# UDC-GAC/pRIblast

Measured on NVIDIA B200. Metric: db-step accessibility throughput, higher is better.
Workload: dtype f32

## Files before the change

### priblast_b200/csrc/acc_kernels.cu

```cuda
#include <cuda_runtime.h>
#include <nvtx3/nvToolsExt.h>

#include <algorithm>
#include <cstdio>
#include <cstdlib>
#include <cstring>
#include <new>
#include <numeric>
#include <string>
#include <vector>

#include "../../include/priblast_acc.h"
#include "acc_core.h"
#include "acc_exact.h"
#include "acc_tables.h"
#include "acc_tile.h"
#include "acc_wide.h"

using namespace prib;

namespace {

struct NvtxRange {
  explicit NvtxRange(const char *name) { nvtxRangePushA(name); }
  ~NvtxRange() { nvtxRangePop(); }
};

constexpr int kThreads = 128;
constexpr int kScanWarps = 4;
constexpr int kFp32MaxSpan = kMaxSpan;
#ifndef PRIB_TC32
#define PRIB_TC32 640
#endif
#ifndef PRIB_TC64
#define PRIB_TC64 288
#endif
template <typename real> struct TileChain { static constexpr bool value = sizeof(real) == 4 && PRIB_CHAIN != 0; };
template <typename real> struct TileMaxThreads { static constexpr int value = sizeof(real) == 4 ? PRIB_TC32 : PRIB_TC64; };

constexpr int kProgBytes = 128 + 16;
template <typename real>
__host__ __device__ constexpr size_t tile_smem_bytes() {
  return ((size_t)kTilePad + (size_t)kTileRows * TileMaxThreads<real>::value) * sizeof(real) +
         (Core<real>::kHotBytes + TileMaxThreads<real>::value + kMaxSpan + 16 + 15) / 16 * 16
         + kProgBytes;
}

__device__ __forceinline__ unsigned smem_u32(const void *p) { return (unsigned)__cvta_generic_to_shared(p); }
__device__ __forceinline__ void tma_bar_init(unsigned long long *bar, unsigned count) {
  asm volatile("mbarrier.init.shared::cta.b64 [%0], %1;" ::"r"(smem_u32(bar)), "r"(count) : "memory");
  asm volatile("fence.mbarrier_init.release.cluster;" ::: "memory");
}
__device__ __forceinline__ void tma_bar_expect(unsigned long long *bar, unsigned bytes) {
  asm volatile("mbarrier.arrive.expect_tx.shared::cta.b64 _, [%0], %1;" ::"r"(smem_u32(bar)), "r"(bytes) : "memory");
}
__device__ __forceinline__ void tma_bar_wait(unsigned long long *bar, unsigned parity) {
  asm volatile(
      "{\n"
      ".reg .pred p;\n"
      "TMA_WAIT:\n"
      "mbarrier.try_wait.parity.shared::cta.b64 p, [%0], %1;\n"
// ... 28 lines not shown
    asm volatile("st.volatile.shared.b32 [%0], %1;" ::"r"((unsigned)__cvta_generic_to_shared(prog + warp)), "r"(value) : "memory");
}
__device__ __forceinline__ void prog_wait_smem(const int *prog, int warp, int need) {
  const unsigned addr = (unsigned)__cvta_generic_to_shared(prog + warp);
  int v;
  do {
    asm volatile("ld.volatile.shared.b32 %0, [%1];" : "=r"(v) : "r"(addr) : "memory");
  } while (v < need);
}
#else
__device__ __forceinline__ void prog_signal_smem(int *prog, int warp, int lane, int value) { prog_signal(prog, warp, lane, value); }
__device__ __forceinline__ void prog_wait_smem(const int *prog, int warp, int need) { prog_wait(prog, warp, need); }
#endif
struct StepSignal {
  int *prog;
  int warp, lane, value;
  bool release;
  __device__ __forceinline__ void operator()() const {
    if (release) prog_signal(prog, warp, lane, value);
    else prog_signal_smem(prog, warp, lane, value);
  }
};

template <typename real, int PAR >
__global__ void __launch_bounds__(TileMaxThreads<real>::value, 1)
k_inside_tile(typename Core<real>::Ctx c, int TX, long long ntiles, real *scratch) {
  constexpr bool CH = TileChain<real>::value;
  typedef Tile<real> TL;
  constexpr int TC = TileMaxThreads<real>::value;
  extern __shared__ __align__(16) unsigned char smem_raw[];
  const int t = threadIdx.x, W = c.W, warp = t >> 5, lane = t & 31;
  constexpr int NW = TC / 32;
  real *base = reinterpret_cast<real *>(smem_raw) + kTilePad;
  unsigned char *stab = smem_raw + ((size_t)kTilePad + (size_t)kTileRows * TC) * sizeof(real);
  uint8_t *sS = stab + Core<real>::kHotBytes;
  const typename Core<real>::SmallTables &T = *reinterpret_cast<const typename Core<real>::SmallTables *>(stab);
  real *scrM1 = scratch + (size_t)blockIdx.x * 2 * (W + 4) * TC;
  real *scrM2 = scrM1 + (size_t)(W + 4) * TC;
  const typename TL::InSmem sm = TL::carve_in(base, TC, sS);
  const int dfirst = TL::first_group(W);
  int *prog = reinterpret_cast<int *>(smem_raw + tile_smem_bytes<real>() - kProgBytes);
  if (t < 32) prog[t] = 0;
  {
    unsigned long long *tbar = reinterpret_cast<unsigned long long *>(prog + 32);
    if (t == 0) {
      tma_bar_init(tbar, 1);
      tma_bar_expect(tbar, (unsigned)Core<real>::kHotBytes);
      tma_copy_g2s(stab, c.T, (unsigned)Core<real>::kHotBytes, tbar);
    }
    __syncthreads();
    tma_bar_wait(tbar, 0);
  }
  int ebase = 0;
  __syncthreads();
  for (long long tile = blockIdx.x; tile < ntiles; tile += gridDim.x) {
    typename TL::Geo ge;
    ge.g0 = tile * TX;
    ge.TC = TC;
    ge.TX = TX;
    ge.H = W + 1;
    __syncthreads();
    for (int k = t; k < kTileRows * TC; k += TC) base[k] = 0;
    for (int k = t; k < TC + 8; k += TC) sS[k] = (ge.g0 + k < c.NC) ? c.S[ge.g0 + k] : 0;
    typename TL::ColState cs;
    TL::col_state(c, ge.g0 + t, cs);
    __syncthreads();
    int ev = ebase, grp = 0;
    typename TL::Chain ch;
    if constexpr (CH) TL::clear(ch);
    for (int d0 = dfirst; d0 <= W + 1; d0 += kTT, ++grp) {
      real gs[kTT], mb[kTT], bs[kTT];
      real *xch = sm.xch + (grp & 1) * kTT * TC;
      if (warp + 1 < NW) prog_wait(prog, warp + 1, ev);
      if constexpr (CH) {
        if (warp >= 2) prog_wait(prog, warp - 2, ev - kEvPerGroup);
        TL::template inside_deep_chain<PAR, TC>(T, ge, sm, scrM1, scrM2, t, d0, ch, xch, mb, bs);
      } else {
        TL::template inside_deep<TC>(T, ge, sm, scrM1, scrM2, t, d0, gs, mb, bs);
      }
      prog_signal_smem(prog, warp, lane, ++ev);
#pragma unroll
      for (int k = 0; k < kTT; ++k) {
        ++ev;
        if (d0 + k >= kTurn) {
          if ((k > 0 || CH) && warp + 1 < NW) prog_wait_smem(prog, warp + 1, ev - 1);
          if (CH && warp + 2 < NW) prog_wait_smem(prog, warp + 2, ev - 1 - k);
          if (warp > 0) prog_wait_smem(prog, warp - 1, ev - kEvSlackIn);
          TL::template inside_shallow<TC>(c, T, ge, sm, scrM1, scrM2, t, cs, d0 + k, CH ? xch[k * TC + t] : gs[k], mb[k],
                                          bs[k], StepSignal{prog, warp, lane, ev, k == kTT - 1});
        } else {
          prog_signal(prog, warp, lane, ev);
        }
      }
    }
    ebase = ev;
  }
}

template <typename real>
__global__ void __launch_bounds__(TileMaxThreads<real>::value, 1)
k_outside_tile(typename Core<real>::Ctx c, int TX, long long ntiles, real *scratch) {
  constexpr bool CH = TileChain<real>::value;
  typedef Tile<real> TL;
  constexpr int TC = TileMaxThreads<real>::value;
  extern __shared__ __align__(16) unsigned char smem_raw[];
  const int t = threadIdx.x, W = c.W, warp = t >> 5, lane = t & 31;
  constexpr int NW = TC / 32;
  real *pad = reinterpret_cast<real *>(smem_raw);
  real *base = pad + kTilePad;
  unsigned char *stab = smem_raw + ((size_t)kTilePad + (size_t)kTileRows * TC) * sizeof(real);
  const typename Core<real>::SmallTables &T = *reinterpret_cast<const typename Core<real>::SmallTables *>(stab);
  uint8_t *sS = stab + Core<real>::kHotBytes;
  real *scrBif = scratch + (size_t)blockIdx.x * 2 * (W + 4) * TC;
  const typename TL::OutSmem sm = TL::carve_out(base, TC, sS);
  const int dlast = TL::first_group(W);
  int *prog = reinterpret_cast<int *>(smem_raw + tile_smem_bytes<real>() - kProgBytes);
  if (t < 32) prog[t] = 0;
  {
    unsigned long long *tbar = reinterpret_cast<unsigned long long *>(prog + 32);
    if (t == 0) {
      tma_bar_init(tbar, 1);
      tma_bar_expect(tbar, (unsigned)Core<real>::kHotBytes);
      tma_copy_g2s(stab, c.T, (unsigned)Core<real>::kHotBytes, tbar);
    }
    __syncthreads();
    tma_bar_wait(tbar, 0);
  }
  int ebase = 0;
  __syncthreads();
  for (long long tile = blockIdx.x; tile < ntiles; tile += gridDim.x) {
    typename TL::Geo ge;
    ge.g0 = tile * TX;
    ge.TC = TC;
    ge.TX = TX;
    ge.H = W + 1;
    __syncthreads();
    for (int k = t; k < kTilePad + kTileRows * TC; k += TC) pad[k] = 0;
    for (int k = t; k < TC + W + kOutBaseTail; k += TC) {
      const long long col = ge.g0 - ge.H - kOutBaseLead + k;
      sS[k] = (col >= 0 && col < c.NC) ? c.S[col] : 0;
    }
    typename TL::ColState cs;
    TL::col_state(c, ge.g0 - ge.H + t, cs);
    __syncthreads();
    int slot = (W + 1) % kRingOut;
    int ev = ebase, grp = 0;
    typename TL::Chain ch;
    if constexpr (CH) TL::clear(ch);
    for (int d0 = W + 1; d0 >= dlast + kTT - 1; d0 -= kTT, ++grp) {
      typename TL::OutDeep o;
      real *xch = sm.xch + (grp & 1) * kTT * TC;
      if (warp > 0) prog_wait(prog, warp - 1, ev);
      if constexpr (CH) {
        if (warp + 2 < NW) prog_wait(prog, warp + 2, ev - kEvPerGroup);
        TL::template outside_deep_chain<TC>(c, T, ge, sm, scrBif, t, cs, d0, slot, ch, xch, o);
      } else {
        TL::template outside_deep<TC>(c, T, ge, sm, scrBif, t, cs, d0, slot, o);
      }
      prog_signal_smem(prog, warp, lane, ++ev);
#pragma unroll
      for (int k = 0; k < kTT; ++k) {
        ++ev;
        if (d0 - k >= kTurn) {
          if ((k > 0 || CH) && warp > 0) prog_wait_smem(prog, warp - 1, ev - 1);
          if (CH && warp >= 2) prog_wait_smem(prog, warp - 2, ev - 1 - k);
          if (warp + 1 < NW) prog_wait_smem(prog, warp + 1, ev - kEvSlackOut);
          TL::template outside_shallow<TC>(c, T, ge, sm, scrBif, t, cs, d0 - k, slot, CH ? xch[k * TC + t] : o.gs[k],
                                           o.bs[k], o.bm1[k], o.ks[k], StepSignal{prog, warp, lane, ev, k == kTT - 1});
        } else {
          prog_signal(prog, warp, lane, ev);
        }
        slot = slot == 0 ? kRingOut - 1 : slot - 1;
      }
    }
    ebase = ev;
  }
}

template <int BYTES>
__device__ __forceinline__ void cp_async_or_zero(void *smem_dst, const void *gsrc, bool pred) {
  const unsigned dst = (unsigned)__cvta_generic_to_shared(smem_dst);
  const int src_bytes = pred ? BYTES : 0;
  asm volatile("cp.async.ca.shared.global [%0], [%1], %2, %3;" ::"r"(dst), "l"(gsrc), "n"(BYTES), "r"(src_bytes) : "memory");
}

template <typename real, bool ALPHA>
__device__ void warp_scan(const typename Core<real>::Ctx &c, int sq, double *ring, real *wbuf, const double *usm,
                          int lane) {
  const int L = c.seq_len[sq], W = c.W;
  const long long off = c.seq_off[sq];
  const double kBig = Core<real>::kScanBig, kLn2 = 0.6931471805599453094;
// ... 291 lines not shown
}

struct prib_ctx {
  prib_acc_params prm{};
  int W = 70, delta = 5;
  bool use_fp32 = true;
  cudaStream_t own_stream = nullptr, stream = nullptr;
  cudaEvent_t ev0 = nullptr, ev1 = nullptr, evk0 = nullptr, evk1 = nullptr;
  cudaEvent_t evp[PRIB_NUM_PHASES + 1] = {};
  bool phases_pending = false, kernel_timed = true, stage_timed = true;
  struct Pipelined {
    bool on = false, launched = false;
    const char *const *seq = nullptr;
    long long fpos = 0;
  } pipe;
  Engine<float> e32;
  Engine<double> e64;
  ExactEngine *ex = nullptr;
  long long ex_max_cols = 0;
  WideEngine *wide = nullptr;
  float *d_log = nullptr;
  int grid_tiles = 0;
  char *d_tile_scratch = nullptr;
  char *d_state = nullptr;
  long long state_cap_bytes = 0;
  long long state_budget = 0;
  long long budget_default = 0, budget_long = 0;
  void set_budget(long long budget) {
    e64.max_cols = budget / state_bytes_per_column(W, 8) / 32 * 32;
    e32.max_cols = budget / state_bytes_per_column(W, 4) / 32 * 32;
    ex_max_cols = budget / exact_state_bytes_per_column(W) / 32 * 32;
    state_budget = budget;
  }
  std::vector<Batch> batches;
  std::vector<int32_t> seq_len;
  std::vector<long long> seq_pos;
  unsigned char *h_arena = nullptr;
  size_t h_arena_cap = 0, h_arena_used = 0;
  unsigned char *h_meta = nullptr;
  size_t h_meta_cap = 0, h_meta_used = 0;
  size_t n_batches = 0;
  float *d_out = nullptr;
  long long out_floats = 0, out_cap = 0;
  bool staged = false, computed = false;
  float *h_stage = nullptr;
  long long h_stage_floats = 0;
// ... 233 lines not shown
    }
    raw_begin += bytes;
    ++used;
  }
  *n_live = used;
  return PRIB_OK;
}

template <typename real>
int run_batch(prib_ctx *c, const Batch &b, bool timed) {
  Engine<real> &e = engine<real>(c);
  if (timed && settle_phases(c) != PRIB_OK) return PRIB_ECUDA;
  const long long used = state_bytes_per_column(c->W, sizeof(real)) * b.NC;
  if (ensure_state(c, used) != PRIB_OK) return PRIB_ECUDA;
  const typename Core<real>::Ctx k = make_ctx<real>(c, b);
  cudaStream_t st = c->stream;
  if (used > c->cnt.dp_state_bytes_used) c->cnt.dp_state_bytes_used = used;
  if (timed) CU(cudaEventRecord(c->evp[0], st));
  CU(cudaMemsetAsync(b.d_flags, 0, sizeof(int32_t) * (size_t)std::max(b.n, 1), st));
  const unsigned grid = (unsigned)((b.NC + kThreads - 1) / kThreads);
  if (timed) CU(cudaEventRecord(c->evp[1], st));
  NvtxRange nvtx_batch("prib:device_batch");
  nvtxRangePushA("prib:inside");
  const int TX = e.TC - (c->W + 1);
  const long long ntiles = (b.NC + TX - 1) / TX;
  const int tgrid = (int)std::min<long long>(ntiles, c->grid_tiles);
  real *scratch = reinterpret_cast<real *>(c->d_tile_scratch);
  if (Tile<real>::first_group(c->W) & 1) k_inside_tile<real, 1><<<tgrid, e.TC, e.tile_smem, st>>>(k, TX, ntiles, scratch);
  else k_inside_tile<real, 0><<<tgrid, e.TC, e.tile_smem, st>>>(k, TX, ntiles, scratch);
  if (timed) CU(cudaEventRecord(c->evp[2], st));
  nvtxRangePop();
  nvtxRangePushA("prib:outer_scans");
  k_outer_scans_warp<real><<<(2 * b.n + e.scan_warps - 1) / e.scan_warps, 32 * e.scan_warps,
                             (size_t)e.scan_warps * 2 * (c->W + 2) * 32 * sizeof(real), st>>>(k);
  if (timed) CU(cudaEventRecord(c->evp[3], st));
  nvtxRangePop();
  nvtxRangePushA("prib:outside");
  k_outside_tile<real><<<tgrid, e.TC, e.tile_smem, st>>>(k, TX, ntiles, scratch);
  if (timed) CU(cudaEventRecord(c->evp[4], st));
  nvtxRangePop();
  nvtxRangePushA("prib:strand_weights");
  const unsigned bgrid = (unsigned)((b.NC + e.TXb - 1) / e.TXb);
  launch_biloop<real, true>(k, bgrid, e.TXb, e.bi_smem, st);
  if (timed) CU(cudaEventRecord(c->evp[5], st));
  launch_biloop<real, false>(k, bgrid, e.TXb, e.bi_smem, st);
  if (timed) CU(cudaEventRecord(c->evp[6], st));
  nvtxRangePop();
  nvtxRangePushA("prib:finalize");
  k_finalize<real><<<grid, kThreads, 0, st>>>(k);
  if (timed) CU(cudaEventRecord(c->evp[7], st));
  nvtxRangePop();
  CU(cudaGetLastError());
  if (timed) c->phases_pending = true;
  c->cnt.kernel_launches += 6;
  c->cnt.batches += 1;
  return PRIB_OK;
}

ExactBatch exact_batch(prib_ctx *c, const Batch &b) {
  ExactBatch eb;
  eb.NC = b.NC;
// ... 238 lines not shown
  int rc = PRIB_OK;
  if (c->W <= kMaxSpan) {
    rc = setup_engine<double>(c, ScaleSpec(), prop.sharedMemPerBlockOptin, err);
    if (rc != PRIB_OK) return bail(rc == PRIB_EINVAL ? fail(rc, err) : rc);
  }
  if (wide) {
    double klog2 = default_scale_wide().klog2;
    if (const char *e = getenv("PRIB_WIDE_KLOG2")) klog2 = atof(e);
    c->wide = wide_create(c->W, c->delta, klog2, err);
    if (!c->wide) return bail(fail(PRIB_ECUDA, err));
  }
  if (c->use_fp32) {
    ScaleSpec sp32 = default_scale_fp32();
    if (const char *e = getenv("PRIB_KLOG2")) sp32.klog2 = atof(e);
    if (const char *e = getenv("PRIB_ALOG2")) sp32.alog2 = atof(e);
    if (const char *e = getenv("PRIB_BLOG2")) sp32.blog2 = atof(e);
    rc = setup_engine<float>(c, sp32, prop.sharedMemPerBlockOptin, err);
    if (rc != PRIB_OK) return bail(rc == PRIB_EINVAL ? fail(rc, err) : rc);
  }
  if (params->mode == 2 || wide) {
    c->ex = exact_create(c->W, c->delta, err);
    if (!c->ex) return bail(fail(PRIB_ECUDA, err));
  }
  const size_t scr64 = (size_t)2 * (c->W + 4) * c->e64.TC * sizeof(double);
  const size_t scr32 = (size_t)2 * (c->W + 4) * c->e32.TC * sizeof(float);
  if (!wide) CUB(cudaMalloc(&c->d_tile_scratch, (size_t)c->grid_tiles * std::max(scr64, scr32)));

  size_t free_b = 0, total_b = 0;
  CUB(cudaMemGetInfo(&free_b, &total_b));
  long long budget = params->max_batch_bytes > 0 ? params->max_batch_bytes
                                                 : std::min<long long>((long long)(free_b * 0.6), 32LL << 30);
  if (budget > (long long)(free_b * 0.9)) budget = (long long)(free_b * 0.9);
  c->budget_long = params->max_batch_bytes > 0 ? budget : std::max<long long>(budget, (long long)(free_b * 0.6));
  c->budget_default = budget;
  c->e64.max_cols = budget / state_bytes_per_column(c->W, 8) / 32 * 32;
  if (c->e64.max_cols < 4096) return bail(fail(PRIB_ECUDA, "device memory budget too small for the DP state"));
  c->set_budget(budget);
#undef CUB
  *out = c;
  return PRIB_OK;
}

void prib_acc_destroy(prib_ctx *c) {
  if (!c) return;
  cudaSetDevice(c->prm.device);
  free_batches(c);
  cudaFree(c->d_state);
  cudaFree(c->d_tile_scratch);
  c->e32.release();
  c->e64.release();
  exact_destroy(c->ex);
  wide_destroy(c->wide);
  cudaFree(c->d_log);
  if (c->h_stage) cudaFreeHost(c->h_stage);
  if (c->h_arena) cudaFreeHost(c->h_arena);
  if (c->h_meta) cudaFreeHost(c->h_meta);
  if (c->h_flags) cudaFreeHost(c->h_flags);
  if (c->h_bad) cudaFreeHost(c->h_bad);
  cudaFree(c->d_bad);
  if (c->ev0) cudaEventDestroy(c->ev0);
  if (c->ev1) cudaEventDestroy(c->ev1);
  if (c->evk0) cudaEventDestroy(c->evk0);
  if (c->evk1) cudaEventDestroy(c->evk1);
  for (auto &e : c->evp)
    if (e) cudaEventDestroy(e);
  if (c->own_stream) cudaStreamDestroy(c->own_stream);
  delete c;
}

int prib_acc_set_stream(prib_ctx *c, void *cuda_stream) {
  if (!c) return fail(PRIB_EINVAL, "null context");
// ... 313 lines not shown
```

### priblast_b200/csrc/acc_tile.h

```cpp
#pragma once
#include <string.h>
#include "acc_core.h"

#ifndef PRIB_CHAIN
#define PRIB_CHAIN 0
#endif

namespace prib {

enum {
  kTT = 4,
  kRingIn = 32,
  kRingOut = 34,
  kRingStem = 8,
  kRingSE = 8,
  kRingMu = 4,
  kXchRows = 2 * 4,
  kTileRows = 88 + (PRIB_CHAIN ? kXchRows : 0),
  kTilePad = 64,
  kOutBaseLead = 2,
  kOutBaseTail = 8,
};

PRIB_HD void prefetch_l1(const void *p) {
#if defined(__CUDA_ARCH__) && defined(PRIB_PREFETCH)
  asm volatile("prefetch.global.L1 [%0];" ::"l"(p));
#else
  (void)p;
#endif
}
enum { kPfDist = 6 };

#if defined(__CUDA_ARCH__)
__device__ __forceinline__ void ffma2_bcast(unsigned long long &acc, float v, float2 g) {
  unsigned long long vv, gg;
  asm("mov.b64 %0, {%1, %1};" : "=l"(vv) : "f"(v));
  asm("mov.b64 %0, {%1, %2};" : "=l"(gg) : "f"(g.x), "f"(g.y));
  asm("fma.rn.f32x2 %0, %1, %2, %0;" : "+l"(acc) : "l"(vv), "l"(gg));
}
__device__ __forceinline__ void unpack2(unsigned long long p, float &lo, float &hi) {
  asm("mov.b64 {%0, %1}, %2;" : "=f"(lo), "=f"(hi) : "l"(p));
}
__device__ __forceinline__ unsigned long long pack2f(float lo, float hi) {
  unsigned long long p;
// ... 5 lines not shown
  asm("fma.rn.f32x2 %0, %1, %2, %0;" : "+l"(acc) : "l"(pack2f(a0, a1)), "l"(pack2f(b0, b1)));
  unpack2(acc, d0, d1);
}
__device__ __forceinline__ void add2(float &s0, float &s1, float a0, float a1, float b) {
  unsigned long long r;
  asm("add.rn.f32x2 %0, %1, %2;" : "=l"(r) : "l"(pack2f(a0, a1)), "l"(pack2f(b, b)));
  unpack2(r, s0, s1);
}
#endif

struct NoStepHook {
  PRIB_HD void operator()() const {}
};

template <typename real>
struct Tile {
  typedef Core<real> K;
  typedef typename K::Ctx Ctx;
  typedef typename K::SmallTables ST;

  struct Geo {
    long long g0;
    int TC, TX, H;
  };

  struct ColState {
    int sq;
    int L, i;
    long long zcol;
  };

  static PRIB_HD void col_state(const Ctx &c, long long g, ColState &cs) {
    cs.sq = -1;
    cs.L = 0;
    cs.i = -1;
    cs.zcol = 0;
    if (g < 0 || g >= c.NC) return;
    const int sq = c.col_seq[g];
    if (sq < 0) return;
    cs.sq = sq;
    cs.L = c.seq_len[sq];
    cs.i = (int)(g - c.seq_off[sq]);
    cs.zcol = c.seq_off[sq] + cs.L;
  }

  static PRIB_HD constexpr int in_cidx(int u1, int sum) {
// ... 9 lines not shown
  static float tf32_trunc(float v) {
    uint32_t b;
    memcpy(&b, &v, 4);
    b &= 0xFFFFE000u;
    memcpy(&v, &b, 4);
    return v;
  }
#endif
  static PRIB_HD real stencil_mul(real w, real v) {
#if !defined(__CUDA_ARCH__)
    if (sizeof(real) == 4 && emu_tf32()) {
      const float wh = tf32_trunc((float)w), wl = tf32_trunc((float)w - wh);
      const float vh = tf32_trunc((float)v), vl = tf32_trunc((float)v - vh);
      return (real)((wh * vh + wl * vh) + wh * vl);
    }
#endif
    return w * v;
  }
  static PRIB_HD real gsel(int k, real g0, real g1, real g2, real g3, real g4, real g5, real g6) {
    return k == 0 ? g0 : k == 1 ? g1 : k == 2 ? g2 : k == 3 ? g3 : k == 4 ? g4 : k == 5 ? g5 : g6;
  }

  static PRIB_HD int first_group(int W) { return W + 2 - ((W + 2 - kTurn + kTT - 1) / kTT) * kTT; }

  struct InSmem {
    real *stemI, *stemB, *stem, *se, *mu, *m2, *xch;
    const uint8_t *S;
  };
  static PRIB_HD InSmem carve_in(real *base, int TC, const uint8_t *S) {
    InSmem s;
    s.stemI = base;
    s.stemB = s.stemI + kRingIn * TC;
    s.stem = s.stemB + kRingIn * TC;
    s.se = s.stem + kRingStem * TC;
    s.mu = s.se + kRingSE * TC;
    s.m2 = s.mu + kRingMu * TC;
    s.xch = s.m2 + kRingMu * TC;
    s.S = S;
    return s;
  }
  struct OutSmem {
    real *stemO, *stemB, *stem, *mu, *m2, *xch;
    const uint8_t *S;
  };
  static PRIB_HD OutSmem carve_out(real *base, int TC, const uint8_t *S) {
    OutSmem s;
    s.S = S;
    s.stemO = base;
    s.stemB = s.stemO + kRingOut * TC;
    s.stem = s.stemB + kRingOut * TC;
    s.mu = s.stem + kRingStem * TC;
    s.m2 = s.mu + kRingMu * TC;
    s.xch = s.m2 + kRingMu * TC;
    return s;
  }

  enum { kChainN = kMaxLoop - 4 + 1 };
  struct Chain {
    real f[2][kChainN];
  };
  static PRIB_HD void clear(Chain &ch) {
#pragma unroll
    for (int a = 0; a < 2; ++a)
#pragma unroll
      for (int b = 0; b < kChainN; ++b) ch.f[a][b] = 0;
  }
  template <int s, int FILE_, int DIR>
  static PRIB_HD real chain_step(const real *e, const real *cg, Chain &ch) {
    real v;
    if constexpr (s == 4) {
      v = cg[2] * (e[DIR * 1] + e[DIR * 3]);
      ch.f[FILE_][0] = v + cg[0] * e[DIR * 2];
    } else if constexpr (s == 5) {
      v = cg[3] * (e[DIR * 1] + e[DIR * 4]) + cg[1] * (e[DIR * 2] + e[DIR * 3]);
      ch.f[FILE_][1] = v;
    } else {
      v = ch.f[FILE_][s - 6] + cg[s - 2 < 6 ? s - 2 : 6] * (e[DIR * 1] + e[DIR * (s - 1)]);
      ch.f[FILE_][s - 4] = v;
    }
// ... 129 lines not shown
        for (int j = 0; j < kTT; ++j) {
          if (m + j <= d0 + kTT - 1 - 5) {
#pragma unroll
            for (int k = 0; k < kTT; ++k)
              if (m + j <= d0 + k - 5) mb[k] += ta[j] * tb[j][k];
          }
        }
      }
    }
  }

  template <int TCC = 0>
  static PRIB_HD void inside_deep(const ST &T, const Geo &ge, const InSmem &sm, const real *scrM1, const real *scrM2,
                                  int t, int d0, real (&gs)[kTT], real (&mb)[kTT], real (&bs)[kTT]) {
    const int TC = TCC > 0 ? TCC : ge.TC;
    const real *cf = K::cf_tab(T), *bu = K::bulge_tab(T);
    const real g0 = T.cg[0], g1 = T.cg[1], g2 = T.cg[2], g3 = T.cg[3], g4 = T.cg[4], g5 = T.cg[5], g6 = T.cg[6];
#pragma unroll
    for (int k = 0; k < kTT; ++k) gs[k] = mb[k] = bs[k] = 0;
#if defined(PRIB_EXP_NODEEP)
    if (d0 == 1000)
#endif
    in_rows<1, TCC>(sm, TC, t, d0, cf, bu, g0, g1, g2, g3, g4, g5, g6, gs, bs);
    in_bif_all(scrM1, scrM2, TC, t, d0, mb);
  }

  template <int S, int K, int PAR>
  static PRIB_HD void in_chain_cell(const real *rowI, int xb, const real *cf, const real *cg, Chain &ch, real (&gs)[kTT]) {
    constexpr int s = S + K;
    if constexpr (s >= 4 && s <= kMaxLoop) {
      const real v = chain_step<s, (PAR + K) & 1, 1>(rowI + xb - ((PAR + K) >> 1), cg, ch);
      gs[K] += cf[s] * v;
    }
  }
  template <int S, int PAR, int TCC>
  static PRIB_HD void in_chain_rows(const InSmem &sm, int TC, int t, int xb, int d0, const real *cf, const real *bu,
                                    const real *cg, Chain &ch, real (&gs)[kTT], real (&bs)[kTT]) {
    if (d0 - S >= 5) {
      const real *rowI = sm.stemI + ((d0 - S) & (kRingIn - 1)) * (TCC > 0 ? TCC : TC);
      in_chain_cell<S, 0, PAR>(rowI, xb, cf, cg, ch, gs);
      in_chain_cell<S, 1, PAR>(rowI, xb, cf, cg, ch, gs);
      in_chain_cell<S, 2, PAR>(rowI, xb, cf, cg, ch, gs);
      in_chain_cell<S, 3, PAR>(rowI, xb, cf, cg, ch, gs);
      const real *rowB = rowI + kRingIn * (TCC > 0 ? TCC : TC) + t;
      const real b0 = rowB[0];
#pragma unroll
      for (int k = 0; k < kTT; ++k)
        if (S + k >= 4 && S + k <= kMaxLoop) bs[k] += bu[S + k] * (rowB[S + k] + b0);
    }
    if constexpr (S > 1) in_chain_rows<S - 1, PAR, TCC>(sm, TC, t, xb, d0, cf, bu, cg, ch, gs, bs);
  }

  template <int PAR, int TCC = 0>
  static PRIB_HD void inside_deep_chain(const ST &T, const Geo &ge, const InSmem &sm, const real *scrM1,
                                        const real *scrM2, int t, int d0, Chain &ch, real *xch, real (&mb)[kTT],
                                        real (&bs)[kTT]) {
    const int TC = TCC > 0 ? TCC : ge.TC;
    const real *cf = K::cf_tab(T), *bu = K::bulge_tab(T), *cg = K::cg_tab(T);
    real gs[kTT];
#pragma unroll
    for (int k = 0; k < kTT; ++k) gs[k] = mb[k] = bs[k] = 0;
    const int xb = t - ((d0 - PAR) >> 1);
    in_chain_rows<kMaxLoop, PAR, TCC>(sm, TC, t, xb, d0, cf, bu, cg, ch, gs, bs);
#pragma unroll
    for (int k = 0; k < kTT; ++k) {
      const int x = xb - ((PAR + k) >> 1);
      if (x >= 0) xch[k * TC + x] = gs[k];
    }
    in_bif_all(scrM1, scrM2, TC, t, d0, mb);
  }

  template <int TCC = 0, typename Hook = NoStepHook>
  static PRIB_HD void inside_shallow(const Ctx &c, const ST &T, const Geo &ge, const InSmem &sm, real *scrM1,
                                     real *scrM2, int t, const ColState &cs, int d, real gs, real mb, real bs,
                                     Hook stores_done = Hook()) {
    const int TC = TCC > 0 ? TCC : ge.TC;
    const real *bu = K::bulge_tab(T);
    real stem = 0, stemI = 0, stemB = 0, stemD = 0, se = 0, mu = 0, m1 = 0, m2 = 0;
    const int smax = imin(kMaxLoop, d - 5);
    const int L = cs.L, i = cs.i, j = i + d;
#if defined(PRIB_EXP_NOSHALLOW)
    const bool live = i >= 0 && j <= L && t + d <= TC - 1 && d == 1000;
#else
    const bool live = i >= 0 && j <= L && t + d <= TC - 1;
#endif
    if (live) {
      const uint8_t *s = sm.S + t;
      const int si = s[0], si1 = s[1], sj = s[d], sj1 = s[d + 1];
      const int te = (j != L) ? T.bp[si][sj1] : 0;
      real p11 = 0, p21a = 0, p21b = 0, p22 = 0;
#if defined(PRIB_EXP_NOTAB)
      if (te && d == 1000) {
#else
      if (te) {
#endif
        const int sd1 = s[d - 1], sd2 = s[d - 2], s2 = s[2], s3 = s[3];
        if (smax >= 2) p11 = c.e_int11[idx11(te, T.bpr[s2][sd1], si1, sj)];
        if (smax >= 3) {
          p21a = c.e_int21[idx21(te, T.bpr[s2][sd2], si1, sd1, sj)];
          p21b = c.e_int21[idx21(T.bpr[s3][sd1], te, sj, si1, s2)];
        }
        if (smax >= 4) p22 = c.e_int22[idx22(te, T.bpr[s3][sd2], si1, s2, sd1, sj)];
      }
      const int tp = T.bp[si1][sj];
      if (tp) {
        const int t2r = T.bpr[s[2]][s[d - 1]];
        stem = K::template scal<K::kScK2>(T) * (sm.se[((d - 2) & (kRingSE - 1)) * TC + t + 1] +
// ... 29 lines not shown
          }
          a += T.tau[te] * bs;
        }
        if (smax >= 3) {
          a += st3[1] * p21a;
          a += st3[2] * p21b;
        }
        if (smax >= 4) {
          a += st4[2] * p22;
          a += T.e_mmI[te][si1][sj] * gs;
        }
        const int tt = T.rt[te];
        a += mu * K::template scal<K::kScMlClose>(T) * T.e_d3[tt][si1] * T.e_d5[tt][sj];
        se = a;
      }
    }
    sm.stemI[(d & (kRingIn - 1)) * TC + t] = stemI;
    sm.stemB[(d & (kRingIn - 1)) * TC + t] = stemB;
    sm.stem[(d & (kRingStem - 1)) * TC + t] = stem;
    sm.se[(d & (kRingSE - 1)) * TC + t] = se;
    sm.mu[(d & (kRingMu - 1)) * TC + t] = mu;
    sm.m2[(d & (kRingMu - 1)) * TC + t] = m2;
#if defined(PRIB_SCR_BEFORE)
    scrM1[d * TC + t] = m1;
    scrM2[d * TC + t] = m2;
#endif
    stores_done();
#if !defined(PRIB_SCR_BEFORE)
    scrM1[d * TC + t] = m1;
    scrM2[d * TC + t] = m2;
#endif
#if defined(PRIB_EXP_NOSTG)
    if (t < ge.TX && i >= 0 && j <= L && d == 1000) {
#else
    if (t < ge.TX && i >= 0 && j <= L) {
#endif
      const long long g = ge.g0 + t;
      if (c.delta == 2) c.put(A_STEM, d, g, stem);
      c.put(A_STEMI, d, g, stemI);
      c.put(A_STEMB, d, g, stemB);
      c.put(A_STEMD, d, g, stemD);
      c.put(A_MULTI, d, g, mu);
      c.put(A_MULTI1, d, g, m1);
      c.put(A_MULTI2, d, g, m2);
      if (!(K::in_safe_range(stem) && K::in_safe_range(se) && K::in_safe_range(mu) && K::in_safe_range(m1) &&
            K::in_safe_range(m2)))
        K::raise_flag(&c.flags[cs.sq], K::range_bits(stem) | K::range_bits(se) | K::range_bits(mu) | K::range_bits(m1) |
                                           K::range_bits(m2));
    }
  }

  static PRIB_HD int wrap_out(int r) { return r >= kRingOut ? r - kRingOut : r; }

  struct OutDeep {
// ... 195 lines not shown
        }
#pragma unroll
        for (int e = 1; e < kTT; ++e) {
          const int mm = W - d0 + e;
          if (p >= 1 && mm >= 5 && mm <= p) {
#pragma unroll
            for (int k = 0; k < kTT; ++k)
              if (k >= e) o.ks[k] += tq[e - 1][k] * tb[e - 1];
          }
        }
      }
    }
  }

  template <int TCC = 0>
  static PRIB_HD void outside_deep(const Ctx &c, const ST &T, const Geo &ge, const OutSmem &sm, const real *scrBif,
                                   int t, const ColState &cs, int d0, int slot_d0 , OutDeep &o) {
    const int TC = TCC > 0 ? TCC : ge.TC, W = c.W;
    const real *bu = K::bulge_tab(T), *cf = K::cf_tab(T);
    const real g0 = T.cg[0], g1 = T.cg[1], g2 = T.cg[2], g3 = T.cg[3], g4 = T.cg[4], g5 = T.cg[5], g6 = T.cg[6];
#pragma unroll
    for (int k = 0; k < kTT; ++k) o.gs[k] = o.bs[k] = o.bm1[k] = o.ks[k] = 0;
    out_rows<1, TCC>(sm, TC, t, d0, slot_d0, W, bu, cf, g0, g1, g2, g3, g4, g5, g6, o);
    out_multi_all(c, ge, scrBif, TC, t, cs, d0, o);
  }

  template <int S, int K>
  static PRIB_HD void out_chain_cell(const real *rowO, int xb, const real *cf, const real *cg, Chain &ch, real (&gs)[kTT]) {
    constexpr int s = S + K - 2;
    if constexpr (s >= 4 && s <= kMaxLoop) {
      const real v = chain_step<s, K & 1, -1>(rowO + xb + (K >> 1) - 1, cg, ch);
      gs[K] += cf[s] * v;
    }
  }
  template <int S, int TCC>
  static PRIB_HD void out_chain_rows(const OutSmem &sm, int TC, int t, int xb, int d0, int slot_d0, int W, const real *bu,
                                     const real *cf, const real *cg, Chain &ch, OutDeep &o) {
    if (d0 + S <= W + 1) {
      const int slot = wrap_out(slot_d0 + S);
      const real *rowO = sm.stemO + slot * (TCC > 0 ? TCC : TC);
      out_chain_cell<S, 0>(rowO, xb, cf, cg, ch, o.gs);
      out_chain_cell<S, 1>(rowO, xb, cf, cg, ch, o.gs);
      out_chain_cell<S, 2>(rowO, xb, cf, cg, ch, o.gs);
      out_chain_cell<S, 3>(rowO, xb, cf, cg, ch, o.gs);
      const real *rowB = sm.stemB + slot * (TCC > 0 ? TCC : TC) + t - 1;
      const real b0 = rowB[0];
#pragma unroll
      for (int k = 0; k < kTT; ++k) {
        const int u = S + k - 2;
        if (u >= 2 && u <= kMaxLoop) o.bs[k] += bu[u] * (rowB[-u] + b0);
      }
    }
    if constexpr (S > 1) out_chain_rows<S - 1, TCC>(sm, TC, t, xb, d0, slot_d0, W, bu, cf, cg, ch, o);
  }

  template <int TCC = 0>
  static PRIB_HD void outside_deep_chain(const Ctx &c, const ST &T, const Geo &ge, const OutSmem &sm, const real *scrBif,
                                         int t, const ColState &cs, int d0, int slot_d0, Chain &ch, real *xch,
                                         OutDeep &o) {
    const int TC = TCC > 0 ? TCC : ge.TC, W = c.W;
    const real *bu = K::bulge_tab(T), *cf = K::cf_tab(T), *cg = K::cg_tab(T);
#pragma unroll
    for (int k = 0; k < kTT; ++k) o.gs[k] = o.bs[k] = o.bm1[k] = o.ks[k] = 0;
    const int xb = t + ((W + 1 - d0) >> 1);
    out_chain_rows<kMaxLoop + 2, TCC>(sm, TC, t, xb, d0, slot_d0, W, bu, cf, cg, ch, o);
#pragma unroll
    for (int k = 0; k < kTT; ++k) {
      const int x = xb + (k >> 1);
      if (x < TC) xch[k * TC + x] = o.gs[k];
    }
    out_multi_all(c, ge, scrBif, TC, t, cs, d0, o);
  }

  template <int TCC = 0, typename Hook = NoStepHook>
  static PRIB_HD void outside_shallow(const Ctx &c, const ST &T, const Geo &ge, const OutSmem &sm, real *scrBif, int t,
                                      const ColState &cs, int d, int slot_d , real gs, real bs,
                                      real bm1, real ks, Hook stores_done = Hook()) {
    const int TC = TCC > 0 ? TCC : ge.TC, W = c.W;
    const real *bu = K::bulge_tab(T);
    real bstem = 0, bstemO = 0, bstemB = 0, bmulti = 0, bmulti2 = 0, bmbif = 0;
    const int smax = imin(kMaxLoop, W - 1 - d);
    const long long g = ge.g0 - ge.H + t;
    const int L = cs.L, p = cs.i, q = p + d;
#if defined(PRIB_EXP_NOSHALLOW)
    const bool live = p >= 0 && q <= L && t + d >= ge.H && d == 1000;
#else
    const bool live = p >= 0 && q <= L && t + d >= ge.H;
#endif
    if (live) {
      const uint8_t *s = sm.S + kOutBaseLead + t;
      const int sp = s[0], sp1 = s[1], sq_ = s[d], sq1 = s[d + 1];
      const bool inner = (p != 0 && q != L);
      const int te = inner ? T.bp[sp][sq1] : 0;
      const int t2_ = T.bp[sp1][sq_];
      double la = 0, lb = 0, lz = 0;
      real p11 = 0, p21a = 0, p21b = 0, p22 = 0;
#if defined(PRIB_EXP_NOTAB)
      if (t2_ && d == 1000) {
#else
      if (t2_) {
#endif
// ... 38 lines not shown
          l += b4[-2] * p11;
          l += T.tau[t2r] * bs;
        }
        if (smax >= 3) {
          l += b5[-2] * p21a;
          l += b5[-3] * p21b;
        }
        if (smax >= 4) {
          l += b6[-3] * p22;
          l += T.e_mmI[t2r][sq1][sp] * gs;
        }
        const real base = (real)exp(la + lb - lz) * dang * T.sB[d];
        bstem = base + K::template scal<K::kScK2>(T) * l + bmulti2 * K::template scal<K::kScMlIntern>(T) * dang;
        bstemO = bstem * T.e_mmI[t2][s[2]][s[d - 1]];
        bstemB = bstem * T.tau[t2];
      }
    }
    sm.stemO[slot_d * TC + t] = bstemO;
    sm.stemB[slot_d * TC + t] = bstemB;
    sm.stem[(d & (kRingStem - 1)) * TC + t] = bstem;
    sm.mu[(d & (kRingMu - 1)) * TC + t] = bmulti;
    sm.m2[(d & (kRingMu - 1)) * TC + t] = bmulti2;
#if defined(PRIB_SCR_BEFORE)
    scrBif[d * TC + t] = bmbif;
#endif
    stores_done();
#if !defined(PRIB_SCR_BEFORE)
    scrBif[d * TC + t] = bmbif;
#endif
#if defined(PRIB_EXP_NOSTG)
    if (t >= ge.H && p >= 0 && q <= L && d == 1000) {
#else
    if (t >= ge.H && p >= 0 && q <= L) {
#endif
      c.put(B_STEM, d, g, bstem);
      c.put(B_STEMO, d, g, bstemO);
      c.put(B_STEMB, d, g, bstemB);
      c.put(B_MULTI, d, g, bmulti);
      c.put(B_MULTI2, d, g, bmulti2);
      if (!(K::in_safe_range(bstem) && K::in_safe_range(bmulti) && K::in_safe_range(bmulti2) &&
            K::in_safe_range(bmbif)))
        K::raise_flag(&c.flags[cs.sq], 4 * (K::range_bits(bstem) | K::range_bits(bmulti) | K::range_bits(bmulti2) |
                                                K::range_bits(bmbif)));
    }
  }
};

}

namespace prib {

template <typename real>
// ... 403 lines not shown
```

Baseline: 94.53 million.

## Carry halo state between consecutive tiles in contiguous per-CTA strips

Each CTA now walks a contiguous strip of columns instead of striding tiles across the grid. Each tile after the first reuses halo values that the previous tile saved to a small global carry buffer, so it needs a halo of only kHaloW columns instead of W+1. The aim is to cut redundant halo recomputation and widen the useful tile width. The cost is extra carry stores and loads, a scratch shift with CTA syncs, and a dedicated warp that replays the halo. The non-first tiles also load more sequence bytes into shared memory.

```diff
diff --git a/priblast_b200/csrc/acc_kernels.cu b/priblast_b200/csrc/acc_kernels.cu
--- a/priblast_b200/csrc/acc_kernels.cu
+++ b/priblast_b200/csrc/acc_kernels.cu
@@ -37,6 +37,7 @@
 #endif
 template <typename real> struct TileChain { static constexpr bool value = sizeof(real) == 4 && PRIB_CHAIN != 0; };
 template <typename real> struct TileMaxThreads { static constexpr int value = sizeof(real) == 4 ? PRIB_TC32 : PRIB_TC64; };
+template <typename real> struct TileCarry { static constexpr bool value = !TileChain<real>::value && !PRIB_HALO_COLD; };
 
 constexpr int kProgBytes = 128 + 16;
 template <typename real>
@@ -111,12 +112,17 @@
   }
 };
 
+struct CtaSync {
+  __device__ __forceinline__ void operator()() const { __syncthreads(); }
+};
+
 template <typename real, int PAR >
 __global__ void __launch_bounds__(TileMaxThreads<real>::value, 1)
-k_inside_tile(typename Core<real>::Ctx c, int TX, long long ntiles, real *scratch) {
-  constexpr bool CH = TileChain<real>::value;
+k_inside_tile(typename Core<real>::Ctx c, Strips sp, real *scratch, real *carry) {
+  constexpr bool CH = TileChain<real>::value, CARRY = TileCarry<real>::value;
   typedef Tile<real> TL;
   constexpr int TC = TileMaxThreads<real>::value;
+  constexpr int SS = TL::scr_stride(TC);
   extern __shared__ __align__(16) unsigned char smem_raw[];
   const int t = threadIdx.x, W = c.W, warp = t >> 5, lane = t & 31;
   constexpr int NW = TC / 32;
@@ -124,8 +130,9 @@
   unsigned char *stab = smem_raw + ((size_t)kTilePad + (size_t)kTileRows * TC) * sizeof(real);
   uint8_t *sS = stab + Core<real>::kHotBytes;
   const typename Core<real>::SmallTables &T = *reinterpret_cast<const typename Core<real>::SmallTables *>(stab);
-  real *scrM1 = scratch + (size_t)blockIdx.x * 2 * (W + 4) * TC;
-  real *scrM2 = scrM1 + (size_t)(W + 4) * TC;
+  real *scrM1 = scratch + (size_t)blockIdx.x * 2 * (W + 4) * SS;
+  real *scrM2 = scrM1 + (size_t)(W + 4) * SS;
+  real *cbuf = carry + (size_t)blockIdx.x * 2 * TL::carry_size(W);
   const typename TL::InSmem sm = TL::carve_in(base, TC, sS);
   const int dfirst = TL::first_group(W);
   int *prog = reinterpret_cast<int *>(smem_raw + tile_smem_bytes<real>() - kProgBytes);
@@ -142,19 +149,55 @@
   }
   int ebase = 0;
   __syncthreads();
-  for (long long tile = blockIdx.x; tile < ntiles; tile += gridDim.x) {
+  const long long ntl = sp.tiles(blockIdx.x);
+  for (long long j = 0; j < ntl; ++j) {
+    const bool warm = CARRY && j > 0;
     typename TL::Geo ge;
-    ge.g0 = tile * TX;
+    ge.g0 = sp.g0_in(blockIdx.x, j);
     ge.TC = TC;
-    ge.TX = TX;
-    ge.H = W + 1;
+    ge.H = warm ? (int)kHaloW : W + 1;
+    ge.TX = TC - ge.H;
     __syncthreads();
     for (int k = t; k < kTileRows * TC; k += TC) base[k] = 0;
-    for (int k = t; k < TC + 8; k += TC) sS[k] = (ge.g0 + k < c.NC) ? c.S[ge.g0 + k] : 0;
+    for (int k = t; k < TC + W + 8; k += TC) sS[k] = (ge.g0 + k < c.NC) ? c.S[ge.g0 + k] : 0;
+    if (warm) TL::scratch_move(scrM1, 2 * (W + 4), SS, ge.TX, 0, W + 1, t, TC, CtaSync());
     typename TL::ColState cs;
     TL::col_state(c, ge.g0 + t, cs);
     __syncthreads();
     int ev = ebase, grp = 0;
+    if (warm && warp == NW - 1) {
+      const real *cget = cbuf + ((j + 1) & 1) * TL::carry_size(W);
+      real cur[kTT][kInCarry], nxt[kTT][kInCarry];
+      auto load = [&](int d0) {
+#pragma unroll
+        for (int k = 0; k < kTT; ++k) {
+          if (d0 + k >= kTurn) TL::in_halo_load(cget, W, d0 + k, lane, nxt[k]);
+        }
+      };
+      load(dfirst);
+      for (int d0 = dfirst; d0 <= W + 1; d0 += kTT) {
+#pragma unroll
+        for (int k = 0; k < kTT; ++k)
+#pragma unroll
+          for (int a = 0; a < kInCarry; ++a) cur[k][a] = nxt[k][a];
+        if (d0 + kTT <= W + 1) load(d0 + kTT);
+        prog_signal_smem(prog, warp, lane, ++ev);
+#pragma unroll
+        for (int k = 0; k < kTT; ++k) {
+          ++ev;
+          if (d0 + k >= kTurn) {
+            prog_wait_smem(prog, warp - 1, ev - kEvSlackIn);
+            TL::in_halo_put(sm, TC, t, d0 + k, cur[k]);
+            StepSignal{prog, warp, lane, ev, k == kTT - 1}();
+          } else {
+            prog_signal(prog, warp, lane, ev);
+          }
+        }
+      }
+      ebase = ev;
+      continue;
+    }
+    real *cput = (CARRY && warp == 0 && j + 1 < ntl) ? cbuf + (j & 1) * TL::carry_size(W) : nullptr;
     typename TL::Chain ch;
     if constexpr (CH) TL::clear(ch);
     for (int d0 = dfirst; d0 <= W + 1; d0 += kTT, ++grp) {
@@ -176,7 +219,7 @@
           if (CH && warp + 2 < NW) prog_wait_smem(prog, warp + 2, ev - 1 - k);
           if (warp > 0) prog_wait_smem(prog, warp - 1, ev - kEvSlackIn);
           TL::template inside_shallow<TC>(c, T, ge, sm, scrM1, scrM2, t, cs, d0 + k, CH ? xch[k * TC + t] : gs[k], mb[k],
-                                          bs[k], StepSignal{prog, warp, lane, ev, k == kTT - 1});
+                                          bs[k], cput, StepSignal{prog, warp, lane, ev, k == kTT - 1});
         } else {
           prog_signal(prog, warp, lane, ev);
         }
@@ -188,10 +231,11 @@
 
 template <typename real>
 __global__ void __launch_bounds__(TileMaxThreads<real>::value, 1)
-k_outside_tile(typename Core<real>::Ctx c, int TX, long long ntiles, real *scratch) {
-  constexpr bool CH = TileChain<real>::value;
+k_outside_tile(typename Core<real>::Ctx c, Strips sp, real *scratch, real *carry) {
+  constexpr bool CH = TileChain<real>::value, CARRY = TileCarry<real>::value;
   typedef Tile<real> TL;
   constexpr int TC = TileMaxThreads<real>::value;
+  constexpr int SS = TL::scr_stride(TC);
   extern __shared__ __align__(16) unsigned char smem_raw[];
   const int t = threadIdx.x, W = c.W, warp = t >> 5, lane = t & 31;
   constexpr int NW = TC / 32;
@@ -200,7 +244,8 @@
   unsigned char *stab = smem_raw + ((size_t)kTilePad + (size_t)kTileRows * TC) * sizeof(real);
   const typename Core<real>::SmallTables &T = *reinterpret_cast<const typename Core<real>::SmallTables *>(stab);
   uint8_t *sS = stab + Core<real>::kHotBytes;
-  real *scrBif = scratch + (size_t)blockIdx.x * 2 * (W + 4) * TC;
+  real *scr = scratch + (size_t)blockIdx.x * 2 * (W + 4) * SS;
+  real *cbuf = carry + (size_t)blockIdx.x * 2 * TL::carry_size(W);
   const typename TL::OutSmem sm = TL::carve_out(base, TC, sS);
   const int dlast = TL::first_group(W);
   int *prog = reinterpret_cast<int *>(smem_raw + tile_smem_bytes<real>() - kProgBytes);
@@ -217,23 +262,64 @@
   }
   int ebase = 0;
   __syncthreads();
-  for (long long tile = blockIdx.x; tile < ntiles; tile += gridDim.x) {
+  const long long ntl = sp.tiles(blockIdx.x);
+  for (long long j = 0; j < ntl; ++j) {
+    const bool warm = CARRY && j > 0;
     typename TL::Geo ge;
-    ge.g0 = tile * TX;
+    ge.g0 = sp.g0_out(blockIdx.x, j);
     ge.TC = TC;
-    ge.TX = TX;
-    ge.H = W + 1;
+    ge.H = warm ? (int)kHaloW : W + 1;
+    ge.TX = TC - ge.H;
+    real *scrBif = scr + TL::out_scr_off(ge, W);
     __syncthreads();
     for (int k = t; k < kTilePad + kTileRows * TC; k += TC) pad[k] = 0;
     for (int k = t; k < TC + W + kOutBaseTail; k += TC) {
       const long long col = ge.g0 - ge.H - kOutBaseLead + k;
       sS[k] = (col >= 0 && col < c.NC) ? c.S[col] : 0;
     }
+    if (warm) {
+      const int dst = TL::out_scr_off(ge, W) + ge.H - W;
+      TL::scratch_move(scr, W + 4, SS, dst, dst + (j == 1 ? sp.TXc : sp.TXw), W, t, TC, CtaSync());
+    }
     typename TL::ColState cs;
     TL::col_state(c, ge.g0 - ge.H + t, cs);
     __syncthreads();
     int slot = (W + 1) % kRingOut;
     int ev = ebase, grp = 0;
+    if (warm && warp == 0) {
+      const real *cget = cbuf + ((j + 1) & 1) * TL::carry_size(W);
+      real cur[kTT][kOutCarry], nxt[kTT][kOutCarry];
+      auto load = [&](int d0) {
+#pragma unroll
+        for (int k = 0; k < kTT; ++k) {
+          if (d0 - k >= kTurn) TL::out_halo_load(cget, W, d0 - k, lane, nxt[k]);
+        }
+      };
+      load(W + 1);
+      for (int d0 = W + 1; d0 >= dlast + kTT - 1; d0 -= kTT) {
+#pragma unroll
+        for (int k = 0; k < kTT; ++k)
+#pragma unroll
+          for (int a = 0; a < kOutCarry; ++a) cur[k][a] = nxt[k][a];
+        if (d0 - kTT >= dlast + kTT - 1) load(d0 - kTT);
+        prog_signal_smem(prog, warp, lane, ++ev);
+#pragma unroll
+        for (int k = 0; k < kTT; ++k) {
+          ++ev;
+          if (d0 - k >= kTurn) {
+            prog_wait_smem(prog, warp + 1, ev - kEvSlackOut);
+            TL::out_halo_put(sm, TC, t, d0 - k, slot, cur[k]);
+            StepSignal{prog, warp, lane, ev, k == kTT - 1}();
+          } else {
+            prog_signal(prog, warp, lane, ev);
+          }
+          slot = slot == 0 ? kRingOut - 1 : slot - 1;
+        }
+      }
+      ebase = ev;
+      continue;
+    }
+    real *cput = (CARRY && warp == NW - 1 && j + 1 < ntl) ? cbuf + (j & 1) * TL::carry_size(W) : nullptr;
     typename TL::Chain ch;
     if constexpr (CH) TL::clear(ch);
     for (int d0 = W + 1; d0 >= dlast + kTT - 1; d0 -= kTT, ++grp) {
@@ -255,7 +341,7 @@
           if (CH && warp >= 2) prog_wait_smem(prog, warp - 2, ev - 1 - k);
           if (warp + 1 < NW) prog_wait_smem(prog, warp + 1, ev - kEvSlackOut);
           TL::template outside_shallow<TC>(c, T, ge, sm, scrBif, t, cs, d0 - k, slot, CH ? xch[k * TC + t] : o.gs[k],
-                                           o.bs[k], o.bm1[k], o.ks[k], StepSignal{prog, warp, lane, ev, k == kTT - 1});
+                                           o.bs[k], o.bm1[k], o.ks[k], cput, StepSignal{prog, warp, lane, ev, k == kTT - 1});
         } else {
           prog_signal(prog, warp, lane, ev);
         }
@@ -593,6 +679,7 @@
   float *d_log = nullptr;
   int grid_tiles = 0;
   char *d_tile_scratch = nullptr;
+  char *d_halo_carry = nullptr;
   char *d_state = nullptr;
   long long state_cap_bytes = 0;
   long long state_budget = 0;
@@ -872,12 +959,11 @@
   if (timed) CU(cudaEventRecord(c->evp[1], st));
   NvtxRange nvtx_batch("prib:device_batch");
   nvtxRangePushA("prib:inside");
-  const int TX = e.TC - (c->W + 1);
-  const long long ntiles = (b.NC + TX - 1) / TX;
-  const int tgrid = (int)std::min<long long>(ntiles, c->grid_tiles);
-  real *scratch = reinterpret_cast<real *>(c->d_tile_scratch);
-  if (Tile<real>::first_group(c->W) & 1) k_inside_tile<real, 1><<<tgrid, e.TC, e.tile_smem, st>>>(k, TX, ntiles, scratch);
-  else k_inside_tile<real, 0><<<tgrid, e.TC, e.tile_smem, st>>>(k, TX, ntiles, scratch);
+  int tgrid = 0;
+  const Strips sp = Strips::make(b.NC, c->grid_tiles, e.TC, c->W, TileCarry<real>::value, &tgrid);
+  real *scratch = reinterpret_cast<real *>(c->d_tile_scratch), *carry = reinterpret_cast<real *>(c->d_halo_carry);
+  if (Tile<real>::first_group(c->W) & 1) k_inside_tile<real, 1><<<tgrid, e.TC, e.tile_smem, st>>>(k, sp, scratch, carry);
+  else k_inside_tile<real, 0><<<tgrid, e.TC, e.tile_smem, st>>>(k, sp, scratch, carry);
   if (timed) CU(cudaEventRecord(c->evp[2], st));
   nvtxRangePop();
   nvtxRangePushA("prib:outer_scans");
@@ -886,7 +972,7 @@
   if (timed) CU(cudaEventRecord(c->evp[3], st));
   nvtxRangePop();
   nvtxRangePushA("prib:outside");
-  k_outside_tile<real><<<tgrid, e.TC, e.tile_smem, st>>>(k, TX, ntiles, scratch);
+  k_outside_tile<real><<<tgrid, e.TC, e.tile_smem, st>>>(k, sp, scratch, carry);
   if (timed) CU(cudaEventRecord(c->evp[4], st));
   nvtxRangePop();
   nvtxRangePushA("prib:strand_weights");
@@ -1171,9 +1257,12 @@
     c->ex = exact_create(c->W, c->delta, err);
     if (!c->ex) return bail(fail(PRIB_ECUDA, err));
   }
-  const size_t scr64 = (size_t)2 * (c->W + 4) * c->e64.TC * sizeof(double);
-  const size_t scr32 = (size_t)2 * (c->W + 4) * c->e32.TC * sizeof(float);
-  if (!wide) CUB(cudaMalloc(&c->d_tile_scratch, (size_t)c->grid_tiles * std::max(scr64, scr32)));
+  const size_t scr64 = (size_t)2 * (c->W + 4) * Tile<double>::scr_stride(c->e64.TC) * sizeof(double);
+  const size_t scr32 = (size_t)2 * (c->W + 4) * Tile<float>::scr_stride(c->e32.TC) * sizeof(float);
+  if (!wide) {
+    CUB(cudaMalloc(&c->d_tile_scratch, (size_t)c->grid_tiles * std::max(scr64, scr32)));
+    CUB(cudaMalloc(&c->d_halo_carry, (size_t)c->grid_tiles * 2 * Tile<double>::carry_size(c->W) * sizeof(double)));
+  }
 
   size_t free_b = 0, total_b = 0;
   CUB(cudaMemGetInfo(&free_b, &total_b));
@@ -1196,6 +1285,7 @@
   free_batches(c);
   cudaFree(c->d_state);
   cudaFree(c->d_tile_scratch);
+  cudaFree(c->d_halo_carry);
   c->e32.release();
   c->e64.release();
   exact_destroy(c->ex);
diff --git a/priblast_b200/csrc/acc_tile.h b/priblast_b200/csrc/acc_tile.h
--- a/priblast_b200/csrc/acc_tile.h
+++ b/priblast_b200/csrc/acc_tile.h
@@ -4,6 +4,9 @@
 
 #ifndef PRIB_CHAIN
 #define PRIB_CHAIN 0
+#endif
+#ifndef PRIB_HALO_COLD
+#define PRIB_HALO_COLD 0
 #endif
 
 namespace prib {
@@ -20,6 +23,35 @@
   kTilePad = 64,
   kOutBaseLead = 2,
   kOutBaseTail = 8,
+  kHaloW = 32,
+  kInCarry = 6,
+  kOutCarry = 5,
+};
+
+struct Strips {
+  int TXc, TXw;
+  long long R, a;
+  PRIB_HD long long cols(long long n) const { return n > 0 ? TXc + (n - 1) * TXw : 0; }
+  PRIB_HD long long tiles(long long b) const { return b < a ? R : R - 1; }
+  PRIB_HD long long start(long long b) const { return b < a ? b * cols(R) : a * cols(R) + (b - a) * cols(R - 1); }
+  PRIB_HD long long g0_in(long long b, long long j) const { return start(b) + cols(tiles(b)) - TXc - j * TXw; }
+  PRIB_HD long long g0_out(long long b, long long j) const { return start(b) + (j > 0 ? TXc + (j - 1) * TXw : 0); }
+  static Strips make(long long NC, int ncta, int TC, int W, bool carry, int *ctas) {
+    Strips s;
+    s.TXc = TC - (W + 1);
+    s.TXw = carry ? TC - kHaloW : s.TXc;
+    if (NC <= (long long)ncta * s.TXc) {
+      s.R = 1;
+      s.a = NC > 0 ? (NC + s.TXc - 1) / s.TXc : 0;
+      *ctas = (int)s.a;
+    } else {
+      const long long per = (long long)ncta * s.TXw;
+      s.R = 1 + (NC - (long long)ncta * s.TXc + per - 1) / per;
+      s.a = (NC - ncta * s.cols(s.R - 1) + s.TXw - 1) / s.TXw;
+      *ctas = ncta;
+    }
+    return s;
+  }
 };
 
 PRIB_HD void prefetch_l1(const void *p) {
@@ -71,6 +103,7 @@
   struct Geo {
     long long g0;
     int TC, TX, H;
+    int SS = 0;
   };
 
   struct ColState {
@@ -126,6 +159,23 @@
   }
 
   static PRIB_HD int first_group(int W) { return W + 2 - ((W + 2 - kTurn + kTT - 1) / kTT) * kTT; }
+
+  static PRIB_HD constexpr int scr_stride(int TC) { return TC - kHaloW + (kMaxSpan + 1 + 31) / 32 * 32; }
+  template <int TCC>
+  static PRIB_HD int scr_ss(const Geo &ge) { return TCC > 0 ? scr_stride(TCC) : ge.SS > 0 ? ge.SS : ge.TC; }
+  static PRIB_HD int out_scr_off(const Geo &ge, int W) { return (W + 1 + 31) / 32 * 32 - ge.H; }
+  template <typename Sync>
+  static PRIB_HD void scratch_move(real *scr, int rows, int SS, int dst, int src, int n, int tid, int nthr, Sync sync) {
+    const int dist = dst < src ? src - dst : dst - src;
+    for (int a = 0; a < n; a += dist) {
+      const int w = imin(dist, n - a), o = dst < src ? a : n - a - w;
+      for (int k = tid; k < rows * w; k += nthr) {
+        const int r = k / w, x = o + k % w;
+        scr[(long long)r * SS + dst + x] = scr[(long long)r * SS + src + x];
+      }
+      sync();
+    }
+  }
 
   struct InSmem {
     real *stemI, *stemB, *stem, *se, *mu, *m2, *xch;
@@ -159,6 +209,33 @@
     return s;
   }
 
+  static PRIB_HD long long carry_size(int W) { return (long long)kInCarry * (W + 2) * kHaloW; }
+  template <typename P>
+  static PRIB_HD P *carry_row(P *cb, int W, int a, int d) { return cb + ((long long)a * (W + 2) + d) * kHaloW; }
+  static PRIB_HD void in_halo_load(const real *cb, int W, int d, int x, real (&v)[kInCarry]) {
+#pragma unroll
+    for (int a = 0; a < kInCarry; ++a) v[a] = carry_row(cb, W, a, d)[x];
+  }
+  static PRIB_HD void in_halo_put(const InSmem &sm, int TC, int t, int d, const real (&v)[kInCarry]) {
+    sm.stemI[(d & (kRingIn - 1)) * TC + t] = v[0];
+    sm.stemB[(d & (kRingIn - 1)) * TC + t] = v[1];
+    sm.stem[(d & (kRingStem - 1)) * TC + t] = v[2];
+    sm.se[(d & (kRingSE - 1)) * TC + t] = v[3];
+    sm.mu[(d & (kRingMu - 1)) * TC + t] = v[4];
+    sm.m2[(d & (kRingMu - 1)) * TC + t] = v[5];
+  }
+  static PRIB_HD void out_halo_load(const real *cb, int W, int d, int x, real (&v)[kOutCarry]) {
+#pragma unroll
+    for (int a = 0; a < kOutCarry; ++a) v[a] = carry_row(cb, W, a, d)[x];
+  }
+  static PRIB_HD void out_halo_put(const OutSmem &sm, int TC, int t, int d, int slot_d, const real (&v)[kOutCarry]) {
+    sm.stemO[slot_d * TC + t] = v[0];
+    sm.stemB[slot_d * TC + t] = v[1];
+    sm.stem[(d & (kRingStem - 1)) * TC + t] = v[2];
+    sm.mu[(d & (kRingMu - 1)) * TC + t] = v[3];
+    sm.m2[(d & (kRingMu - 1)) * TC + t] = v[4];
+  }
+
   enum { kChainN = kMaxLoop - 4 + 1 };
   struct Chain {
     real f[2][kChainN];
@@ -334,7 +411,7 @@
     if (d0 == 1000)
 #endif
     in_rows<1, TCC>(sm, TC, t, d0, cf, bu, g0, g1, g2, g3, g4, g5, g6, gs, bs);
-    in_bif_all(scrM1, scrM2, TC, t, d0, mb);
+    in_bif_all(scrM1, scrM2, scr_ss<TCC>(ge), t, d0, mb);
   }
 
   template <int S, int K, int PAR>
@@ -379,22 +456,22 @@
       const int x = xb - ((PAR + k) >> 1);
       if (x >= 0) xch[k * TC + x] = gs[k];
     }
-    in_bif_all(scrM1, scrM2, TC, t, d0, mb);
+    in_bif_all(scrM1, scrM2, scr_ss<TCC>(ge), t, d0, mb);
   }
 
   template <int TCC = 0, typename Hook = NoStepHook>
   static PRIB_HD void inside_shallow(const Ctx &c, const ST &T, const Geo &ge, const InSmem &sm, real *scrM1,
                                      real *scrM2, int t, const ColState &cs, int d, real gs, real mb, real bs,
-                                     Hook stores_done = Hook()) {
-    const int TC = TCC > 0 ? TCC : ge.TC;
+                                     real *carry = nullptr, Hook stores_done = Hook()) {
+    const int TC = TCC > 0 ? TCC : ge.TC, SS = scr_ss<TCC>(ge);
     const real *bu = K::bulge_tab(T);
     real stem = 0, stemI = 0, stemB = 0, stemD = 0, se = 0, mu = 0, m1 = 0, m2 = 0;
     const int smax = imin(kMaxLoop, d - 5);
     const int L = cs.L, i = cs.i, j = i + d;
 #if defined(PRIB_EXP_NOSHALLOW)
-    const bool live = i >= 0 && j <= L && t + d <= TC - 1 && d == 1000;
+    const bool live = i >= 0 && j <= L && (t < ge.TX || t + d <= TC - 1) && d == 1000;
 #else
-    const bool live = i >= 0 && j <= L && t + d <= TC - 1;
+    const bool live = i >= 0 && j <= L && (t < ge.TX || t + d <= TC - 1);
 #endif
     if (live) {
       const uint8_t *s = sm.S + t;
@@ -470,14 +547,19 @@
     sm.mu[(d & (kRingMu - 1)) * TC + t] = mu;
     sm.m2[(d & (kRingMu - 1)) * TC + t] = m2;
 #if defined(PRIB_SCR_BEFORE)
-    scrM1[d * TC + t] = m1;
-    scrM2[d * TC + t] = m2;
+    scrM1[d * SS + t] = m1;
+    scrM2[d * SS + t] = m2;
 #endif
     stores_done();
 #if !defined(PRIB_SCR_BEFORE)
-    scrM1[d * TC + t] = m1;
-    scrM2[d * TC + t] = m2;
-#endif
+    scrM1[d * SS + t] = m1;
+    scrM2[d * SS + t] = m2;
+#endif
+    if (carry) {
+      const real v[kInCarry] = {stemI, stemB, stem, se, mu, m2};
+#pragma unroll
+      for (int a = 0; a < kInCarry; ++a) carry_row(carry, c.W, a, d)[t] = v[a];
+    }
 #if defined(PRIB_EXP_NOSTG)
     if (t < ge.TX && i >= 0 && j <= L && d == 1000) {
 #else
@@ -719,7 +801,7 @@
 #pragma unroll
     for (int k = 0; k < kTT; ++k) o.gs[k] = o.bs[k] = o.bm1[k] = o.ks[k] = 0;
     out_rows<1, TCC>(sm, TC, t, d0, slot_d0, W, bu, cf, g0, g1, g2, g3, g4, g5, g6, o);
-    out_multi_all(c, ge, scrBif, TC, t, cs, d0, o);
+    out_multi_all(c, ge, scrBif, scr_ss<TCC>(ge), t, cs, d0, o);
   }
 
   template <int S, int K>
@@ -766,14 +848,14 @@
       const int x = xb + (k >> 1);
       if (x < TC) xch[k * TC + x] = o.gs[k];
     }
-    out_multi_all(c, ge, scrBif, TC, t, cs, d0, o);
+    out_multi_all(c, ge, scrBif, scr_ss<TCC>(ge), t, cs, d0, o);
   }
 
   template <int TCC = 0, typename Hook = NoStepHook>
   static PRIB_HD void outside_shallow(const Ctx &c, const ST &T, const Geo &ge, const OutSmem &sm, real *scrBif, int t,
                                       const ColState &cs, int d, int slot_d , real gs, real bs,
-                                      real bm1, real ks, Hook stores_done = Hook()) {
-    const int TC = TCC > 0 ? TCC : ge.TC, W = c.W;
+                                      real bm1, real ks, real *carry = nullptr, Hook stores_done = Hook()) {
+    const int TC = TCC > 0 ? TCC : ge.TC, W = c.W, SS = scr_ss<TCC>(ge);
     const real *bu = K::bulge_tab(T);
     real bstem = 0, bstemO = 0, bstemB = 0, bmulti = 0, bmulti2 = 0, bmbif = 0;
     const int smax = imin(kMaxLoop, W - 1 - d);
@@ -858,12 +940,17 @@
     sm.mu[(d & (kRingMu - 1)) * TC + t] = bmulti;
     sm.m2[(d & (kRingMu - 1)) * TC + t] = bmulti2;
 #if defined(PRIB_SCR_BEFORE)
-    scrBif[d * TC + t] = bmbif;
+    scrBif[d * SS + t] = bmbif;
 #endif
     stores_done();
 #if !defined(PRIB_SCR_BEFORE)
-    scrBif[d * TC + t] = bmbif;
-#endif
+    scrBif[d * SS + t] = bmbif;
+#endif
+    if (carry) {
+      const real v[kOutCarry] = {bstemO, bstemB, bstem, bmulti, bmulti2};
+#pragma unroll
+      for (int a = 0; a < kOutCarry; ++a) carry_row(carry, W, a, d)[t - (TC - kHaloW)] = v[a];
+    }
 #if defined(PRIB_EXP_NOSTG)
     if (t >= ge.H && p >= 0 && q <= L && d == 1000) {
 #else
diff --git a/profiles/halo_carry_summary.py b/profiles/halo_carry_summary.py
--- /dev/null
+++ b/profiles/halo_carry_summary.py
@@ -0,0 +1,40 @@
+import glob
+import json
+import os
+import sys
+
+import numpy as np
+
+
+def main(d):
+    runs = {"carry": [], "cold": []}
+    for v in runs:
+        for f in sorted(glob.glob(os.path.join(d, f"bench_{v}_*.json"))):
+            r = json.load(open(f))
+            r["_run"] = os.path.basename(f)
+            runs[v].append(r)
+    print(open(os.path.join(d, "gpu.csv")).read().strip())
+    for v, rs in runs.items():
+        for r in rs:
+            ph = r["roofline"]["phase_ms_per_step"]
+            print(f"{r['_run']}: value {r['value']:.4e} nt/s, ms_per_step {r['ms_per_step']:.1f}, phases "
+                  + ", ".join(f"{k} {x:.1f}" for k, x in ph.items()))
+        ms = [r["ms_per_step"] for r in rs]
+        print(f"{v}: ms_per_step mean {np.mean(ms):.1f}, spread (max - min) {max(ms) - min(ms):.1f}")
+        for k in rs[0]["roofline"]["phase_ms_per_step"]:
+            x = [r["roofline"]["phase_ms_per_step"][k] for r in rs]
+            print(f"  {k}: mean {np.mean(x):.1f}, spread {max(x) - min(x):.1f}")
+    a, b = runs["carry"][0], runs["cold"][0]
+    for name in ("acc.npy", "cond.npy"):
+        same = all(np.array_equal(np.load(os.path.join(d, f"dump_{v}_{k}", name)),
+                                  np.load(os.path.join(d, f"dump_cold_1", name)))
+                   for v in runs for k in range(1, len(runs[v]) + 1))
+        print(f"{name} bit-identical across all runs: {same}")
+    cs = {r["e2e"]["checksum"] for rs in runs.values() for r in rs}
+    print(f"e2e.checksum equal across all runs: {len(cs) == 1} ({sorted(cs)})")
+    print(f"parity carry: {json.dumps(a['parity'])}")
+    print(f"parity cold:  {json.dumps(b['parity'])}")
+
+
+if __name__ == "__main__":
+    main(sys.argv[1])
```

After: 93.47 million (median of 6 runs). -1.1%, worse.
